# struan-robertson/shoeprint-image-retrieval

Hardware: AMD Instinct MI355X
Metric: query x gallery NCC pairs/sec (higher is better)
Workload: dtype f32; 1 GPU; config 2: WVU2019-shaped VGG16 conv3_3 NCC: Q=100 x G=1500 (1500/GPU), features [256,128,64] stored as float32, rotations/scales none, queries signal 1 / noise 126; method=fft, gallery_chunk=1500, storage=float32, parallelism=gallery-shard x1, streams=1

## Files before the change

shoeprint-image-retrieval_amd/csrc/ncc_pair6.hip:

```cpp
#include <cstdlib>

#include "fft_core.h"
#include "ncc_fft_cfg.h"

namespace spr {
namespace {

#ifndef SPR_ABL
#define SPR_ABL 0
#endif
#ifndef SPR_X6
#define SPR_X6 0
#endif
#ifdef SPR_STAMPS
constexpr int kStampPoints = 12, kStampChannels = 8, kStampFirst = 8;
__device__ unsigned long long g_stamps[12 * kStampChannels * kStampPoints];
#define SPR_STAMP(i) st[i] = __builtin_amdgcn_s_memtime()
#else
#define SPR_STAMP(i)
#endif

constexpr int kTileQ6 = 16, kTileG6 = 16;

struct Pair6Args {
  int channels, nq, ng;
  int ih, iw;
  int inv_per_chan;
  int accumulate;
  int tile0;
  int tiles_g;
  int prio_mode;
  unsigned q_flags_off, g_flags_off;
};

template <int DIR>
__device__ __forceinline__ void pfa12(cf (&x)[12]) {
  constexpr float h = DIR > 0 ? 0.86602540378443860f : -0.86602540378443860f;
  cf a[3][4];
#pragma unroll
  for (int n2 = 0; n2 < 4; ++n2) {
    const cf x0 = x[(3 * n2) % 12], x1 = x[(4 + 3 * n2) % 12], x2 = x[(8 + 3 * n2) % 12];
    const cf s = x1 + x2, d = x1 - x2;
    const cf m = x0 - 0.5f * s;
    a[0][n2] = x0 + s;
    a[1][n2] = pk_iaxpy_u(d, h, m);
    a[2][n2] = pk_iaxpy_u(d, -h, m);
  }
#pragma unroll
  for (int k1 = 0; k1 < 3; ++k1) {
    const cf e0 = a[k1][0] + a[k1][2], e1 = a[k1][0] - a[k1][2];
    const cf o0 = a[k1][1] + a[k1][3], o1 = a[k1][1] - a[k1][3];
    x[(4 * k1) % 12] = e0 + o0;
    x[(4 * k1 + 18) % 12] = e0 - o0;
    x[(4 * k1 + 9) % 12] = DIR > 0 ? pk_add_i(e1, o1) : pk_sub_i(e1, o1);
    x[(4 * k1 + 27) % 12] = DIR > 0 ? pk_sub_i(e1, o1) : pk_add_i(e1, o1);
  }
}

template <class C>
struct Six {
  static_assert(C::SIX == 1 && C::EH == 12 && C::TGH == 16 && C::NW == 96 && C::NT == 384, "192 x 96 on six waves");
  static constexpr int NT = C::NT, WAVES = NT / 64;
  static constexpr int RS = 139;
  static __device__ __forceinline__ int xpos(int u) {
    if (SPR_X6 == 0) return (u / 21) * RS + u % 21;
    const int a = u < 21 ? 0 : (u < 32 ? 1 : (u < 43 ? 2 : (u < 53 ? 1 : 2)));
    const int o = u < 21 ? u : (u < 32 ? u - 11 : (u < 43 ? u - 22 : (u < 53 ? u - 43 : (u == 53 ? 9 : u - 54))));
    return a * RS + o;
  }
  static constexpr int XR = 65;
  static constexpr int XROWS = 6;
  static constexpr int kXbWave = XROWS * XR + 6;
  static constexpr int kImgOff = 0;
  static constexpr int kImgBytes = C::COLS * RS * 8;
  static constexpr int kXbOff = kImgOff + kImgBytes;
  static constexpr int kNyqOff = kXbOff + WAVES * kXbWave * 8;
  static constexpr int kHalfBytes = kNyqOff + 2 * 2 * C::NH * 8;
  static constexpr int kRedOff = 2 * kHalfBytes;
  static constexpr int kPeakOff = kRedOff + 128;
  static constexpr int kTwOff = kPeakOff + 64;
  static constexpr int kCtabOff = kTwOff + C::NH * 8;
  static constexpr int kListOff = kCtabOff + 48 * 4;
  static constexpr int kLdsBytes = kListOff;
  static_assert(kLdsBytes + 2 * 2 * 1024 <= 160 * 1024, "one workgroup of two pairs per CU, up to 1024 channels");
  static_assert(kXbOff % 8 == 0 && kNyqOff % 8 == 0 && kHalfBytes % 16 == 0 && kTwOff % 8 == 0 && kCtabOff % 8 == 0, "");
};

template <class C, bool PEAKS>
__global__ void __launch_bounds__(2 * C::NT, 3)
pair6_kernel(Pair6Args g, const unsigned char* __restrict__ pq, size_t q_item_bytes,
             const unsigned char* __restrict__ pg, size_t g_item_bytes, float* __restrict__ scores, long long ld,
             long long col0, float* __restrict__ maps_out, const cf* __restrict__ tw_h,
             const float* __restrict__ ctab, int32_t* __restrict__ peak_yx, int32_t* __restrict__ peak_tag,
             int32_t tag) {
  using S = Six<C>;
  constexpr int NT = S::NT, RS = S::RS, XR = S::XR;
  constexpr int H2 = C::EH / 2;

  constexpr int kWgPerTile = kTileQ6 * kTileG6 / 2;
  const int tile = g.tile0 + static_cast<int>(blockIdx.x) / kWgPerTile;
  const int within = static_cast<int>(blockIdx.x) % kWgPerTile;
  const int tq = tile / g.tiles_g, tg = tile - tq * g.tiles_g;
  const int half = uniform(static_cast<int>(threadIdx.x) >= NT ? 1 : 0);
  const int q_first = tq * kTileQ6 + 2 * (within >> 4);
  const int gi_item = tg * kTileG6 + 2 * (within & 7) + ((within >> 3) & 1);
  if (q_first >= g.nq || gi_item >= g.ng) return;
  const bool live = q_first + half < g.nq;
  const int qi = live ? q_first + half : q_first;

  unsigned char* lds = dyn_lds();
  unsigned char* hl = lds + half * S::kHalfBytes;
  float* red = reinterpret_cast<float*>(lds + S::kRedOff) + half * 8;
  unsigned* bar = reinterpret_cast<unsigned*>(lds + S::kRedOff + 64) + half * 8;
  unsigned* nlive_p = bar + 2;
  unsigned bar_target = 0;
  cf* R = reinterpret_cast<cf*>(hl + S::kImgOff);
  cf* nyq = reinterpret_cast<cf*>(hl + S::kNyqOff);
  cf* twt_h = reinterpret_cast<cf*>(lds + S::kTwOff);
  cf* ctab2 = reinterpret_cast<cf*>(lds + S::kCtabOff);
  unsigned short* chan = reinterpret_cast<unsigned short*>(lds + S::kListOff) + half * g.channels;

  const int tid0 = static_cast<int>(threadIdx.x) - half * NT;
  const int wv = uniform(tid0 >> 6);
  cf* xb = reinterpret_cast<cf*>(hl + S::kXbOff) + wv * S::kXbWave;

  const unsigned char* g_item = pg + static_cast<size_t>(gi_item) * g_item_bytes;
  const unsigned char* q_item = pq + static_cast<size_t>(qi) * q_item_bytes;

  if (tid0 == 0) *bar = 0u;
  if (half == 0) {
    for (int k = tid0; k < C::NH; k += NT) twt_h[k] = cconj(tw_h[(k / C::TGH) * (k % C::TGH)]);
    if (tid0 < 24) {
      const int a = (tid0 / 3) * 2, t = tid0 % 3;
      ctab2[tid0] = cmake(ctab[(3 * a + 16 * t) % 48], ctab[(3 * (a + 1) + 16 * t) % 48]);
    }
  }
  for (int k = tid0; k < g.channels; k += NT)
    chan[k] = (q_item[g.q_flags_off + k] | g_item[g.g_flags_off + k]) ? 0xFFFFu : static_cast<unsigned short>(k);
  __syncthreads();
  if (tid0 == 0) {
    int n = 0;
    for (int k = 0; k < g.channels; ++k) {
      const unsigned short v = chan[k];
      if (v != 0xFFFFu) chan[n++] = v;
    }
    if (n == 0) chan[0] = 0;
    *nlive_p = static_cast<unsigned>(n);
  }
  __syncthreads();
  const int nlive = uniform(static_cast<int>(*nlive_p));
  const int last_i = nlive > 0 ? nlive - 1 : 0;
  auto chan_at = [&](int i) { return static_cast<int>(chan[i < last_i ? i : last_i]); };

  float4 nxt[2 * H2];
  cf nyq_g, nyq_q;
  const BufRsrc g_rs = make_rsrc(g_item, g_item_bytes), q_rs = make_rsrc(q_item, q_item_bytes);
  const unsigned voff16 = static_cast<unsigned>(tid0) * 16u;
  const unsigned voff_nyq = static_cast<unsigned>(tid0 % C::NH) * 8u + C::kNyqOffset * 8u;
  constexpr unsigned kChanBytes = C::kSpecPerChan * 8u;
  const unsigned inv_base = static_cast<unsigned>(g.channels) * kChanBytes;
  auto issue_unit = [&](int c, int rc) {
    const unsigned so = static_cast<unsigned>(c) * kChanBytes + static_cast<unsigned>(rc * H2 * NT * 16);
    if (SPR_ABL == 1) {
      for (int mm = 0; mm < 2 * H2; ++mm) nxt[mm] = make_float4(0.001f * so, 0.5f, 0.25f, 0.125f);
      return;
    }
#pragma unroll
    for (int mm = 0; mm < H2; ++mm) {
      nxt[mm] = buf_ld16(g_rs, voff16, so + mm * NT * 16);
      nxt[H2 + mm] = buf_ld16(q_rs, voff16, so + mm * NT * 16);
    }
  };
  auto issue_nyq = [&](int c) {
    const unsigned so = static_cast<unsigned>(c) * kChanBytes;
    nyq_g = buf_ld8(g_rs, voff_nyq, so);
    nyq_q = buf_ld8(q_rs, voff_nyq, so);
  };
  static_assert(2 * C::NH == NT, "one Nyquist value per lane");

#ifndef SPR_EMU
  {
    const int gw = half * S::WAVES + wv;
    if (g.prio_mode == 2 && (gw == 4 || gw == 5 || gw >= 8)) __builtin_amdgcn_s_setprio(1);
  }
#endif
  cf acc[6][2];
#pragma unroll
  for (int pp = 0; pp < 6; ++pp) acc[pp][0] = acc[pp][1] = cmake(0.0f, 0.0f);

  issue_nyq(chan_at(0));
  nyq[tid0] = tid0 < C::NH ? nyq_g : nyq_q;
  issue_nyq(chan_at(1));
  nyq[NT + tid0] = tid0 < C::NH ? nyq_g : nyq_q;
  issue_unit(chan_at(0), 0);
  __syncthreads();

  for (int ci = 0; ci < nlive; ++ci) {
    const int c = chan_at(ci), c1 = chan_at(ci + 1), c2 = chan_at(ci + 2);
#ifdef SPR_STAMPS
    unsigned long long st[kStampPoints] = {};
#endif
    SPR_STAMP(0);
    const int tid = opaque(tid0);
    const int lane = tid & 63;
    const int g4 = lane >> 4, tc = lane & 15;

    auto product = [&](cf (&z)[12], int rc) {
#pragma unroll
      for (int mm = 0; mm < H2; ++mm) {
        const float4 a = nxt[mm], b = nxt[H2 + mm];
        z[2 * mm] = cmul(cmake(a.x, a.y), cmake(b.x, b.y));
        z[2 * mm + 1] = cmul(cmake(a.z, a.w), cmake(b.z, b.w));
      }
      if (rc == 0 && tid < 16) {
        const cf* nq = nyq + (ci & 1) * NT;
#pragma unroll
        for (int m = 0; m < 12; ++m) {
          const int k1 = tc + 16 * m;
          z[m] = pk_add_i(z[m], cmul(nq[k1], nq[C::NH + k1]));
        }
      }
    };
    auto stage12 = [&](cf (&z)[12]) {
      pfa12<+1>(z);
#pragma unroll
      for (int p = 1; p < 12; ++p) z[p] = cmul(z[p], twt_h[p * 16 + tc]);
    };
    auto exchange = [&](const cf (&z)[12], cf (&y)[16], int rc) {
      const int own0 = (rc * 24 + 4 * wv) * RS;
      const int xb_el = (S::kXbOff - S::kImgOff) / 8 + wv * S::kXbWave;
      const int skew = ((xb_el + 6 - own0) % 32 + 32) % 32;
      cf* own = R + own0 + skew;
      wave_sync();
      cf* w0 = xb + lane;
      cf* w1 = own + lane;
      if (SPR_ABL != 3) {
#pragma unroll
        for (int p = 0; p < 6; ++p) w0[p * XR] = z[p];
#pragma unroll
        for (int p = 6; p < 12; ++p) w1[(p - 6) * XR] = z[p];
      }
      wave_sync();
      const cf* rd = (tc < 6 ? xb + tc * XR : (tc < 12 ? own + (tc - 6) * XR : xb)) + 16 * g4;
#pragma unroll
      for (int tt = 0; tt < 16; ++tt) y[tt] = rd[tt];
    };
    auto part2 = [&](cf (&y)[16], int rc) {
      wave_sync();
      if (tc < 12) {
        if (SPR_ABL != 4) Dft<16, +1>::run(y);
        cf* col = R + (rc * 24 + 4 * wv + g4) * RS + tc;
        if (SPR_ABL != 3) {
#pragma unroll
          for (int s = 0; s < 11; ++s) col[12 * s] = y[s];
        }
      }
    };

    {
      cf za[12], ya[16], zb[12], yb[16];
      issue_nyq(c2);
      product(za, 0);
      issue_unit(c, 1);
      stage12(za);
#pragma unroll
      for (int p = 0; p < 12; ++p) pin(za[p]);
      SPR_STAMP(1);
      bar_target += S::WAVES;
      if (SPR_ABL != 2) group_barrier(bar, bar_target);
      SPR_STAMP(2);
      product(zb, 1);
      sched_fence();
      exchange(za, ya, 0);
      sched_fence();
      stage12(zb);
      sched_fence();
      issue_unit(c1, 0);
      SPR_STAMP(3);
      part2(ya, 0);
      SPR_STAMP(4);
      exchange(zb, yb, 1);
      SPR_STAMP(5);
      part2(yb, 1);
      SPR_STAMP(6);
    }
    bar_target += S::WAVES;
    if (SPR_ABL != 2) group_barrier(bar, bar_target);
    SPR_STAMP(7);
    {
      const int grp = lane / 3;
      const int t3 = lane - 3 * grp;
      const int grp_r = grp < C::kRowGroups ? grp : C::kRowGroups - 1;
      const int row = wv * C::kRowGroups + grp_r;
      const int tm = t3 == 0 ? 0 : 3 - t3;
      const cf* dbase = R + t3 * RS + row;
      const cf* mbase = R + tm * RS + row;
      const cf* cc = ctab2 + t3;
      cf z[16];
#pragma unroll
      for (int a2 = 0; a2 < 8; ++a2) {
        const cf ck = cc[a2 * 3];
#pragma unroll
        for (int h = 0; h < 2; ++h) {
          const int a = 2 * a2 + h;
          const int ra = (3 * a) % 16, rm = (3 * ((16 - a) % 16)) % 16;
          const cf av = dbase[3 * ra * RS];
          const cf bv = mbase[3 * rm * RS];
          cf v = h == 0 ? pk_conj_iaxpy<0>(av, ck, bv) : pk_conj_iaxpy<1>(av, ck, bv);
          if (a == 0) {
            const cf v0 = cmake(av.x + av.y, av.x - av.y);
            v = t3 == 0 ? v0 : v;
          }
          z[a] = v;
        }
      }
      SPR_STAMP(8);
      if (SPR_ABL != 4) Dft<16, +1>::run(z);
      sched_fence();
      float4 iv[6];
      const unsigned so_inv = inv_base + static_cast<unsigned>(c) * static_cast<unsigned>(g.inv_per_chan) * 4u;
#pragma unroll
      for (int pp = 0; pp < 6; ++pp)
        iv[pp] = SPR_ABL == 1 ? make_float4(1.f, 1.f, 1.f, 1.f) : buf_ld16(g_rs, voff16, so_inv + pp * NT * 16);
      const float kH = 0.86602540378443860f;
      const cf kl = t3 == 1 ? cmake(-0.5f, kH) : cmake(1.0f, 0.0f);
      const cf hb = t3 == 0 ? cmake(kH, 0.0f) : cmake(-kH, 0.0f);
      cf* wx = R + S::xpos(lane < 63 ? lane : 62) + wv * C::kRowGroups;
      const cf* rxt[3];
#pragma unroll
      for (int tt = 0; tt < 3; ++tt) rxt[tt] = R + S::xpos(3 * grp_r + tt) + wv * C::kRowGroups;
      wave_sync();
      if (lane < 63 && SPR_ABL != 3) {
#pragma unroll
        for (int r = 0; r < 16; ++r) wx[3 * r * RS] = z[r];
      }
      SPR_STAMP(9);
      wave_sync();
      cf yv[6][3];
#pragma unroll
      for (int pp = 0; pp < 6; ++pp)
#pragma unroll
        for (int tt = 0; tt < 3; ++tt)
          yv[pp][tt] = pp < 5 ? rxt[tt][(9 * pp + 3 * t3) * RS] : rxt[tt][45 * RS];
#pragma unroll
      for (int pp = 0; pp < 6; ++pp) {
        const cf y0 = yv[pp][0], y1 = yv[pp][1], y2 = yv[pp][2];
        const cf s = y1 + y2, d = y1 - y2;
        const cf m = y0 - 0.5f * s;
        const cf ob = pk_iaxpy<0>(d, hb, m);
        const cf oa = pk_iaxpy<1>(d, kl, pk_axpy<0>(s, kl, y0));
        const cf ia = cmake(iv[pp].x, iv[pp].y), ib = cmake(iv[pp].z, iv[pp].w);
        acc[pp][0] = oa * ia + acc[pp][0];
        acc[pp][1] = ob * ib + acc[pp][1];
        if (maps_out && half == 0) {
          const int n1 = t3 + 3 * pp;
          const int real_row = wv * C::kRowGroups + grp;
          if (n1 < 16 && grp < C::kRowGroups && real_row < g.ih) {
            const int ma = t3 == 2 ? n1 + 16 : n1, mb = t3 == 2 ? n1 : n1 + 16;
            float* dst = maps_out + (static_cast<size_t>(c) * g.ih + real_row) * g.iw;
            if (2 * ma < g.iw) dst[2 * ma] = oa.x * ia.x;
            if (2 * ma + 1 < g.iw) dst[2 * ma + 1] = oa.y * ia.y;
            if (2 * mb < g.iw) dst[2 * mb] = ob.x * ib.x;
            if (2 * mb + 1 < g.iw) dst[2 * mb + 1] = ob.y * ib.y;
          }
        }
      }
      nyq[(ci & 1) * NT + tid] = tid < C::NH ? nyq_g : nyq_q;
    }
    SPR_STAMP(10);
#ifdef SPR_STAMPS
    if (blockIdx.x == 777 && (tid0 & 63) == 0 && ci >= kStampFirst && ci < kStampFirst + kStampChannels) {
      for (int i = 0; i < kStampPoints; ++i)
        g_stamps[((half * 6 + wv) * kStampChannels + (ci - kStampFirst)) * kStampPoints + i] = st[i];
    }
#endif
  }

  if constexpr (PEAKS) {
    const int lane = tid0 & 63;
    const int grp = lane / 3, t3 = lane - 3 * grp;
    const int real_row = wv * C::kRowGroups + grp;
    const bool row_ok = grp < C::kRowGroups && real_row < g.ih;
    float best = 0.0f;
    int where = kNoPeak;
#pragma unroll
    for (int pp = 0; pp < 6; ++pp) {
      const int n1 = t3 + 3 * pp;
      const int ma = t3 == 2 ? n1 + 16 : n1, mb = t3 == 2 ? n1 : n1 + 16;
      const int at = real_row << 16;
      if (row_ok && n1 < 16) {
        if (2 * ma < g.iw) peak_take(best, where, acc[pp][0].x, at | (2 * ma));
        if (2 * ma + 1 < g.iw) peak_take(best, where, acc[pp][0].y, at | (2 * ma + 1));
        if (2 * mb < g.iw) peak_take(best, where, acc[pp][1].x, at | (2 * mb));
        if (2 * mb + 1 < g.iw) peak_take(best, where, acc[pp][1].y, at | (2 * mb + 1));
      }
    }
    wave_peak(best, where);
    int* red_pos = reinterpret_cast<int*>(lds + S::kPeakOff) + half * 8;
    if ((tid0 & 63) == 0) {
      red[wv] = best;
      red_pos[wv] = where;
    }
    __syncthreads();
    if (tid0 == 0 && live) {
      float b = red[0];
      int p = red_pos[0];
      for (int w = 1; w < S::WAVES; ++w) peak_take(b, p, red[w], red_pos[w]);
      store_peak(scores, peak_yx, peak_tag, static_cast<size_t>(qi) * ld + col0 + gi_item, b / static_cast<float>(g.channels), p,
                 tag, g.accumulate);
    }
    return;
  }
  float best = 0.0f;
#pragma unroll
  for (int pp = 0; pp < 6; ++pp) {
    best = fmaxf(best, fmaxf(fmaxf(acc[pp][0].x, acc[pp][0].y), fmaxf(acc[pp][1].x, acc[pp][1].y)));
  }
  for (int m = 32; m >= 1; m >>= 1) best = fmaxf(best, shfl_xor(best, m));
  if ((tid0 & 63) == 0) red[wv] = best;
  __syncthreads();
  if (tid0 == 0 && scores && live) {
    float b = red[0];
    for (int w = 1; w < S::WAVES; ++w) b = fmaxf(b, red[w]);
    const float s = b / static_cast<float>(g.channels);
    float* dst = scores + static_cast<size_t>(qi) * ld + col0 + gi_item;
    const float prev = g.accumulate ? *dst : 0.0f;
    *dst = s > prev ? s : prev;
  }
}

using C6 = Cfg<12, 16, 12, 8, 384, 5, 2, 1>;

}

#ifdef SPR_STAMPS
extern "C" int spr_debug_read_stamps(unsigned long long* host, int n) {
  return hipMemcpyFromSymbol(host, HIP_SYMBOL(g_stamps), sizeof(unsigned long long) * n) == hipSuccess ? 0 : -1;
}
#endif

size_t pair6_lds_bytes() { return Six<C6>::kLdsBytes; }
int pair6_max_rows() { return C6::kRows6; }
int pair6_max_cols() { return 64; }

template <bool PEAKS>
static int launch_pair6_t(const NccGeom& g, const PlanScratch& s, const PairCall& c) {
  if (!s.six_ctab) { set_error("pair6_kernel: the plan has no pre-twist table"); return SPR_ERR_ARG; }
  using S = Six<C6>;
  Pair6Args a{};
  a.channels = g.channels; a.nq = static_cast<int>(c.nq); a.ng = static_cast<int>(c.ng);
  a.ih = g.ih; a.iw = g.iw; a.inv_per_chan = g.inv_per_chan; a.accumulate = c.accumulate;
  a.tiles_g = ceil_div(static_cast<int>(c.ng), kTileG6);
  a.q_flags_off = static_cast<unsigned>(sizeof(cf) * static_cast<size_t>(g.channels) * g.spec_per_chan);
  a.g_flags_off = static_cast<unsigned>(static_cast<size_t>(g.channels) * (sizeof(cf) * g.spec_per_chan + sizeof(float) * g.inv_per_chan));
  if (g.channels > 1024) { set_error("pair6_kernel: at most 1024 channels"); return SPR_ERR_UNSUPPORTED; }
  const size_t lds_bytes = S::kLdsBytes + 2 * sizeof(unsigned short) * static_cast<size_t>(g.channels);
  a.prio_mode = env_int("SPR_P6_PRIO", 2);
  const int64_t tiles = static_cast<int64_t>(ceil_div(static_cast<int>(c.nq), kTileQ6)) * a.tiles_g;
  (void)hipFuncSetAttribute(reinterpret_cast<const void*>(pair6_kernel<C6, PEAKS>), hipFuncAttributeMaxDynamicSharedMemorySize,
                            kLdsLimit);
  const int64_t max_tiles = pair_tiles_per_launch(kTileQ6 * kTileG6 / 2, 2 * C6::NT);
  for (int64_t t0 = 0; t0 < tiles; t0 += max_tiles) {
    const int64_t n = tiles - t0 < max_tiles ? tiles - t0 : max_tiles;
    a.tile0 = static_cast<int>(t0);
    hipLaunchKernelGGL(HIP_KERNEL_NAME(pair6_kernel<C6, PEAKS>), dim3(static_cast<unsigned>(n * (kTileQ6 * kTileG6 / 2))), dim3(2 * C6::NT),
                       lds_bytes, c.stream, a, static_cast<const unsigned char*>(c.pq),
                       prepared_query_item_bytes(g, SPR_NCC_FFT), static_cast<const unsigned char*>(c.pg),
                       prepared_gallery_item_bytes(g, SPR_NCC_FFT), c.scores, static_cast<long long>(c.ld),
                       static_cast<long long>(c.col0), c.maps_out, s.tw_h, s.six_ctab, c.peak_yx, c.peak_tag, c.tag);
    const int rc = check_launch("pair6_kernel");
    if (rc != SPR_OK) return rc;
  }
  return SPR_OK;
}

int launch_pair6(const NccGeom& g, const PlanScratch& s, const PairCall& c) {
  if (c.nq == 0 || c.ng == 0) return SPR_OK;
  return c.peak_yx ? launch_pair6_t<true>(g, s, c) : launch_pair6_t<false>(g, s, c);
}

}
```

Baseline: 281,700 pairs/s.

## Parallelise channel compaction, premultiply Nyquist terms, hoist twiddles and channel lookups

Replaces the serial single-thread channel-list compaction with a wave-ballot prefix scan across all threads. The Nyquist products are multiplied once at store time, halving that LDS buffer, and added in a separate step. Twiddle loads are hoisted ahead of the PFA-12, and channel indices are carried in uniform registers instead of being re-read from LDS each iteration. A MAPS template parameter removes the runtime maps_out branch. Together these aim to cut prologue latency and per-channel LDS traffic, at the cost of extra registers and more barriers in the prologue.

```diff
diff --git a/shoeprint-image-retrieval_amd/csrc/ncc_pair6.hip b/shoeprint-image-retrieval_amd/csrc/ncc_pair6.hip
--- a/shoeprint-image-retrieval_amd/csrc/ncc_pair6.hip
+++ b/shoeprint-image-retrieval_amd/csrc/ncc_pair6.hip
@@ -75,7 +75,8 @@
   static constexpr int kImgBytes = C::COLS * RS * 8;
   static constexpr int kXbOff = kImgOff + kImgBytes;
   static constexpr int kNyqOff = kXbOff + WAVES * kXbWave * 8;
-  static constexpr int kHalfBytes = kNyqOff + 2 * 2 * C::NH * 8;
+  static constexpr int kNyqBuf = C::NH;
+  static constexpr int kHalfBytes = kNyqOff + 2 * kNyqBuf * 8;
   static constexpr int kRedOff = 2 * kHalfBytes;
   static constexpr int kPeakOff = kRedOff + 128;
   static constexpr int kTwOff = kPeakOff + 64;
@@ -86,7 +87,7 @@
   static_assert(kXbOff % 8 == 0 && kNyqOff % 8 == 0 && kHalfBytes % 16 == 0 && kTwOff % 8 == 0 && kCtabOff % 8 == 0, "");
 };
 
-template <class C, bool PEAKS>
+template <class C, bool PEAKS, bool MAPS>
 __global__ void __launch_bounds__(2 * C::NT, 3)
 pair6_kernel(Pair6Args g, const unsigned char* __restrict__ pq, size_t q_item_bytes,
              const unsigned char* __restrict__ pg, size_t g_item_bytes, float* __restrict__ scores, long long ld,
@@ -112,7 +113,6 @@
   unsigned char* hl = lds + half * S::kHalfBytes;
   float* red = reinterpret_cast<float*>(lds + S::kRedOff) + half * 8;
   unsigned* bar = reinterpret_cast<unsigned*>(lds + S::kRedOff + 64) + half * 8;
-  unsigned* nlive_p = bar + 2;
   unsigned bar_target = 0;
   cf* R = reinterpret_cast<cf*>(hl + S::kImgOff);
   cf* nyq = reinterpret_cast<cf*>(hl + S::kNyqOff);
@@ -135,20 +135,35 @@
       ctab2[tid0] = cmake(ctab[(3 * a + 16 * t) % 48], ctab[(3 * (a + 1) + 16 * t) % 48]);
     }
   }
-  for (int k = tid0; k < g.channels; k += NT)
-    chan[k] = (q_item[g.q_flags_off + k] | g_item[g.g_flags_off + k]) ? 0xFFFFu : static_cast<unsigned short>(k);
+  int n_before = 0;
+  {
+    int* tot = reinterpret_cast<int*>(red);
+    const int ln = tid0 & 63;
+    for (int k0 = 0; k0 < g.channels; k0 += NT) {
+      const int k = k0 + tid0;
+      const bool alive = k < g.channels && !(q_item[g.q_flags_off + k] | g_item[g.g_flags_off + k]);
+      int lo = alive && ln < 32 ? static_cast<int>(1u << ln) : 0, hi = alive && ln >= 32 ? static_cast<int>(1u << (ln - 32)) : 0;
+      for (int m = 1; m < 64; m <<= 1) {
+        lo |= shfl_xor(lo, m);
+        hi |= shfl_xor(hi, m);
+      }
+      const unsigned below_lo = ln < 32 ? (1u << ln) - 1u : 0xFFFFFFFFu, below_hi = ln < 32 ? 0u : (1u << (ln - 32)) - 1u;
+      const int before = __builtin_popcount(static_cast<unsigned>(lo) & below_lo) + __builtin_popcount(static_cast<unsigned>(hi) & below_hi);
+      if (k0 > 0) __syncthreads();
+      if (ln == 0) tot[wv] = __builtin_popcount(static_cast<unsigned>(lo)) + __builtin_popcount(static_cast<unsigned>(hi));
+      __syncthreads();
+      int at = n_before + before;
+      for (int w = 0; w < S::WAVES; ++w) {
+        const int t = tot[w];
+        at += w < wv ? t : 0;
+        n_before += t;
+      }
+      if (alive) chan[at] = static_cast<unsigned short>(k);
+    }
+    if (n_before == 0 && tid0 == 0) chan[0] = 0;
+  }
   __syncthreads();
-  if (tid0 == 0) {
-    int n = 0;
-    for (int k = 0; k < g.channels; ++k) {
-      const unsigned short v = chan[k];
-      if (v != 0xFFFFu) chan[n++] = v;
-    }
-    if (n == 0) chan[0] = 0;
-    *nlive_p = static_cast<unsigned>(n);
-  }
-  __syncthreads();
-  const int nlive = uniform(static_cast<int>(*nlive_p));
+  const int nlive = uniform(n_before);
   const int last_i = nlive > 0 ? nlive - 1 : 0;
   auto chan_at = [&](int i) { return static_cast<int>(chan[i < last_i ? i : last_i]); };
 
@@ -188,15 +203,19 @@
 #pragma unroll
   for (int pp = 0; pp < 6; ++pp) acc[pp][0] = acc[pp][1] = cmake(0.0f, 0.0f);
 
-  issue_nyq(chan_at(0));
-  nyq[tid0] = tid0 < C::NH ? nyq_g : nyq_q;
-  issue_nyq(chan_at(1));
-  nyq[NT + tid0] = tid0 < C::NH ? nyq_g : nyq_q;
-  issue_unit(chan_at(0), 0);
+  int sc0 = uniform(chan_at(0)), sc1 = uniform(chan_at(1)), sc2 = uniform(chan_at(2));
+  auto store_nyq = [&](int buf, int lane_of_pair) {
+    if (lane_of_pair < C::NH) nyq[buf * S::kNyqBuf + lane_of_pair] = cmul(nyq_g, nyq_q);
+  };
+  issue_nyq(sc0);
+  store_nyq(0, tid0);
+  issue_nyq(sc1);
+  store_nyq(1, tid0);
+  issue_unit(sc0, 0);
   __syncthreads();
 
   for (int ci = 0; ci < nlive; ++ci) {
-    const int c = chan_at(ci), c1 = chan_at(ci + 1), c2 = chan_at(ci + 2);
+    const int c = sc0, c1 = sc1, c2 = sc2;
 #ifdef SPR_STAMPS
     unsigned long long st[kStampPoints] = {};
 #endif
@@ -212,19 +231,26 @@
         z[2 * mm] = cmul(cmake(a.x, a.y), cmake(b.x, b.y));
         z[2 * mm + 1] = cmul(cmake(a.z, a.w), cmake(b.z, b.w));
       }
-      if (rc == 0 && tid < 16) {
-        const cf* nq = nyq + (ci & 1) * NT;
-#pragma unroll
-        for (int m = 0; m < 12; ++m) {
-          const int k1 = tc + 16 * m;
-          z[m] = pk_add_i(z[m], cmul(nq[k1], nq[C::NH + k1]));
-        }
+    };
+    auto add_nyq = [&](cf (&z)[12]) {
+      if (tid < 16) {
+        const cf* nq = nyq + (ci & 1) * S::kNyqBuf + tc;
+        cf pr[12];
+#pragma unroll
+        for (int m = 0; m < 12; ++m) pr[m] = nq[16 * m];
+#pragma unroll
+        for (int m = 0; m < 12; ++m) z[m] = pk_add_i(z[m], pr[m]);
       }
     };
     auto stage12 = [&](cf (&z)[12]) {
+      cf w[12];
+#pragma unroll
+      for (int p = 1; p < 12; ++p) w[p] = twt_h[p * 16 + tc];
+      sched_fence();
       pfa12<+1>(z);
-#pragma unroll
-      for (int p = 1; p < 12; ++p) z[p] = cmul(z[p], twt_h[p * 16 + tc]);
+      sched_fence();
+#pragma unroll
+      for (int p = 1; p < 12; ++p) z[p] = cmul(z[p], w[p]);
     };
     auto exchange = [&](const cf (&z)[12], cf (&y)[16], int rc) {
       const int own0 = (rc * 24 + 4 * wv) * RS;
@@ -262,6 +288,8 @@
       issue_nyq(c2);
       product(za, 0);
       issue_unit(c, 1);
+      sched_fence();
+      add_nyq(za);
       stage12(za);
 #pragma unroll
       for (int p = 0; p < 12; ++p) pin(za[p]);
@@ -315,6 +343,7 @@
         }
       }
       SPR_STAMP(8);
+      const int list_next = chan_at(ci + 3);
       if (SPR_ABL != 4) Dft<16, +1>::run(z);
       sched_fence();
       float4 iv[6];
@@ -352,7 +381,7 @@
         const cf ia = cmake(iv[pp].x, iv[pp].y), ib = cmake(iv[pp].z, iv[pp].w);
         acc[pp][0] = oa * ia + acc[pp][0];
         acc[pp][1] = ob * ib + acc[pp][1];
-        if (maps_out && half == 0) {
+        if (MAPS && half == 0) {
           const int n1 = t3 + 3 * pp;
           const int real_row = wv * C::kRowGroups + grp;
           if (n1 < 16 && grp < C::kRowGroups && real_row < g.ih) {
@@ -365,7 +394,10 @@
           }
         }
       }
-      nyq[(ci & 1) * NT + tid] = tid < C::NH ? nyq_g : nyq_q;
+      store_nyq(ci & 1, tid);
+      sc0 = sc1;
+      sc1 = sc2;
+      sc2 = uniform(list_next);
     }
     SPR_STAMP(10);
 #ifdef SPR_STAMPS
@@ -443,7 +475,7 @@
 int pair6_max_rows() { return C6::kRows6; }
 int pair6_max_cols() { return 64; }
 
-template <bool PEAKS>
+template <bool PEAKS, bool MAPS>
 static int launch_pair6_t(const NccGeom& g, const PlanScratch& s, const PairCall& c) {
   if (!s.six_ctab) { set_error("pair6_kernel: the plan has no pre-twist table"); return SPR_ERR_ARG; }
   using S = Six<C6>;
@@ -457,13 +489,13 @@
   const size_t lds_bytes = S::kLdsBytes + 2 * sizeof(unsigned short) * static_cast<size_t>(g.channels);
   a.prio_mode = env_int("SPR_P6_PRIO", 2);
   const int64_t tiles = static_cast<int64_t>(ceil_div(static_cast<int>(c.nq), kTileQ6)) * a.tiles_g;
-  (void)hipFuncSetAttribute(reinterpret_cast<const void*>(pair6_kernel<C6, PEAKS>), hipFuncAttributeMaxDynamicSharedMemorySize,
+  (void)hipFuncSetAttribute(reinterpret_cast<const void*>(pair6_kernel<C6, PEAKS, MAPS>), hipFuncAttributeMaxDynamicSharedMemorySize,
                             kLdsLimit);
   const int64_t max_tiles = pair_tiles_per_launch(kTileQ6 * kTileG6 / 2, 2 * C6::NT);
   for (int64_t t0 = 0; t0 < tiles; t0 += max_tiles) {
     const int64_t n = tiles - t0 < max_tiles ? tiles - t0 : max_tiles;
     a.tile0 = static_cast<int>(t0);
-    hipLaunchKernelGGL(HIP_KERNEL_NAME(pair6_kernel<C6, PEAKS>), dim3(static_cast<unsigned>(n * (kTileQ6 * kTileG6 / 2))), dim3(2 * C6::NT),
+    hipLaunchKernelGGL(HIP_KERNEL_NAME(pair6_kernel<C6, PEAKS, MAPS>), dim3(static_cast<unsigned>(n * (kTileQ6 * kTileG6 / 2))), dim3(2 * C6::NT),
                        lds_bytes, c.stream, a, static_cast<const unsigned char*>(c.pq),
                        prepared_query_item_bytes(g, SPR_NCC_FFT), static_cast<const unsigned char*>(c.pg),
                        prepared_gallery_item_bytes(g, SPR_NCC_FFT), c.scores, static_cast<long long>(c.ld),
@@ -476,7 +508,8 @@
 
 int launch_pair6(const NccGeom& g, const PlanScratch& s, const PairCall& c) {
   if (c.nq == 0 || c.ng == 0) return SPR_OK;
-  return c.peak_yx ? launch_pair6_t<true>(g, s, c) : launch_pair6_t<false>(g, s, c);
-}
-
-}
+  if (c.peak_yx) return launch_pair6_t<true, false>(g, s, c);
+  return c.maps_out ? launch_pair6_t<false, true>(g, s, c) : launch_pair6_t<false, false>(g, s, c);
+}
+
+}
```

Result: faster. 291,100 pairs/s, median of 6 (+3.3%).
